# VinAIResearch/GaPro

Hardware: AMD Instinct MI355X
Metric: scenes/sec pseudo-label gen (ScanNetV2-train-shaped synthetic scenes) (higher is better)
Workload: dtype f64

## Files before the change

### gapro_amd/csrc/fit_wg.h

```cpp
#pragma once
#include <math.h>

#include <algorithm>
#include <type_traits>

#include "common.h"
#include "fit_layout.h"
#include "fit_math.h"
#include "epilogue.h"

namespace {
using namespace gapro_fit;
using namespace gapro_fit_math;

#ifndef GAPRO_NT
#define GAPRO_NT 512
#endif
constexpr int NT = GAPRO_NT;
constexpr int NW = NT / 64;
constexpr int kMaxMpLds = 512;
constexpr int kMaxDynLds = 150 * 1024;
constexpr int kRedSlots = 8;
constexpr int kTu4MinMp = 320;

using gapro_mfma::d4;



constexpr int kTileDoubles = NW * 16 * 17;
constexpr int kFuseMaxMp = 128;
constexpr int kWgTile = 128;
constexpr int kWgKC = 8;
constexpr int kWgRow = kWgTile + 16;
constexpr int kWgStage = 2 * kWgKC * kWgRow;
constexpr int kWgRingDoubles = 2 * kWgStage;
inline __host__ __device__ int part_doubles(int Mp) { return Mp <= kFuseMaxMp ? 3 * (Mp / 16) * Mp : 0; }
inline __host__ __device__ int scratch_doubles(int Mp) {
  const int a = kRedSlots * NT;
  const int b = Mp * 17 + 64 * 17;
  static_assert(kTileDoubles <= kWgStage, "the transpose tiles alias one stage of the operand ring");
  const int c = Mp <= kFuseMaxMp ? kTileDoubles + part_doubles(Mp) : kWgRingDoubles;
  int m = a > b ? a : b;
  return m > c ? m : c;
}
inline __host__ __device__ long long staged_lds_bytes(int m, int d) {
  const int Mp = gapro_pad_m(m, d);
  return 8LL * (2LL * d * Mp + scratch_doubles(Mp));
}
inline __host__ __device__ bool staged_ok(int m, int d) {
  return gapro_pad_m(m, d) <= kMaxMpLds && d <= 32 && staged_lds_bytes(m, d) <= kMaxDynLds;
}


struct Fit {
  int M, T, D, Mp;
  int M1;
  gd* mat[B_COUNT];
  gd* vec[V_COUNT];
  gd *X, *Z, *mZ, *vZ, *gZ, *Xt, *dinv, *dinvT, *scal;
};

#ifdef GAPRO_PROFILE
constexpr int kProfSlots = 28;
#endif
struct Shared {
  Fit f;
#ifdef GAPRO_PROFILE
  unsigned long long prof[kProfSlots];
  unsigned long long t_last;
  unsigned long long t_start;
#endif
  double red[NW];
  double dblk[16 * 17];
  double dinv[16 * 17];
  double c, rho_s, rho_l, s, ell, inv_l2;
  int status;
  int chol_bad;
};
__shared__ Shared g_sh;

#ifdef GAPRO_PROFILE
__device__ inline void prof_stamp(int id) {
  __syncthreads();
  if (threadIdx.x == 0) {
    const unsigned long long t = wall_clock64();
    g_sh.prof[id] += t - g_sh.t_last;
    g_sh.t_last = t;
  }
}
#else
__device__ inline void prof_stamp(int) {}
#endif

__device__ inline void gh_pair(double y, double mu, double sd, double t, double w, bool want_e, double* E, double* dmu,
                               double* dvar) {
  if (want_e) {
    double lp, r;
    log_ndtr_ratio_erfcx(y * (mu - sd * t), &lp, &r);
    *E += w * lp; *dmu += w * r; *dvar -= w * t * r;
    log_ndtr_ratio_erfcx(y * (mu + sd * t), &lp, &r);
    *E += w * lp; *dmu += w * r; *dvar += w * t * r;
  } else {
    double r = ndtr_ratio(y * (mu - sd * t));
    *dmu += w * r; *dvar -= w * t * r;
    r = ndtr_ratio(y * (mu + sd * t));
    *dmu += w * r; *dvar += w * t * r;
  }
}

__device__ inline int claim_fit(unsigned* ticket) {
  if (!ticket) return blockIdx.x;
  __shared__ int s_claim;
  if (threadIdx.x == 0) s_claim = (int)atomicAdd(ticket, 1u);
  __syncthreads();
  return __builtin_amdgcn_readfirstlane(s_claim);
}

__device__ inline double block_sum(double v) {
  v = wave_sum_shfl(v);
  __syncthreads();
  if ((threadIdx.x & 63) == 0) g_sh.red[threadIdx.x >> 6] = v;
  __syncthreads();
  double t = 0.0;
  for (int w = 0; w < NW; ++w) t += g_sh.red[w];
  return t;
}

__device__ inline double sqdist_t(const ldsd* At, int i, const ldsd* Bt, int j, int D, int Mp) {
  double s = 0.0;
  for (int d = 0; d < D; ++d) {
    const double t = At[d * Mp + i] - Bt[d * Mp + j];
    s += t * t;
  }
  return s;
}

__device__ inline void stage_points_t(ldsd* dst, const gd* src, int n, int D, int Mp) {
  for (int e = threadIdx.x; e < D * Mp; e += NT) {
    const int d = e / Mp, i = e - d * Mp;
    dst[e] = i < n ? src[(size_t)i * D + d] : 0.0;
  }
}

enum { ORD_ROWMAJOR = 0,
       ORD_ROWS_DESC = 1,
       ORD_COLMAJOR = 2,
       ORD_SHELLS = 3 };
typedef double d2 __attribute__((ext_vector_type(2)));
typedef __attribute__((address_space(3))) d2 lds_d2;
typedef __attribute__((address_space(1))) d2 g_d2;

template <int TU, bool SCALE, int KS = 2, int ORD = ORD_ROWMAJOR, bool TRIM = false, int PK = 0, int QK = 0,
          typename KRange, typename Epi>
__device__ __forceinline__ void gemm_tn_body(int mo_tiles, int no_tiles, bool lower_only, const gd* __restrict__ P,
                                          const gd* __restrict__ Q, int ld, const gd* __restrict__ qscale, KRange kr,
                                          Epi epi) {
  mo_tiles = uni(mo_tiles);
  no_tiles = uni(no_tiles);
  lower_only = uni((int)lower_only) != 0;
  ld = uni(ld);
  P = uni_ptr(P);
  Q = uni_ptr(Q);
  qscale = uni_ptr(qscale);
  const int wave = uni(threadIdx.x >> 6), lane = threadIdx.x & 63;
  const int lr = lane & 15, lq = lane >> 4;
  auto tile = [&](auto tv_tag, int i0, int j0) {
    constexpr int TV = decltype(tv_tag)::value;
    constexpr bool MINOR = PK || QK;
    constexpr int KSV = MINOR ? 2 : (TV >= 4 ? 1 : KS), KB = 4 * KSV;
    int klo, khi;
    kr(i0, j0, &klo, &khi);
    klo = uni(klo);
    khi = uni(khi);
    if (TRIM) {
      const int kmax = uni((g_sh.f.M + 7) / 8 * 8);
      khi = khi < kmax ? khi : kmax;
    }
    d4 acc[TV][TV];
#pragma unroll
    for (int u = 0; u < TV; ++u)
#pragma unroll
      for (int v = 0; v < TV; ++v) acc[u][v] = (d4){0.0, 0.0, 0.0, 0.0};
    const gd* pbase = PK ? P + (size_t)(i0 + lr) * ld + 2 * lq : P + (size_t)(MINOR ? 2 * lq : lq) * ld + i0 + lr;
    const gd* qbase = QK ? Q + (size_t)(j0 + lr) * ld + 2 * lq : Q + (size_t)(MINOR ? 2 * lq : lq) * ld + j0 + lr;
    double a0[KSV][TV], b0[KSV][TV], a1[KSV][TV], b1[KSV][TV];
    double s0[KSV], s1[KSV];
    auto load_block = [&](int k, double (&a)[KSV][TV], double (&b)[KSV][TV], double (&sc)[KSV]) {
      if constexpr (MINOR) {
#pragma unroll
        for (int u = 0; u < TV; ++u) {
          if constexpr (PK) {
            const d2 t = *(const g_d2*)(pbase + (size_t)(16 * u) * ld + k);
            a[0][u] = t[0];
            a[1][u] = t[1];
          } else {
            a[0][u] = pbase[(size_t)k * ld + 16 * u];
            a[1][u] = pbase[(size_t)(k + 1) * ld + 16 * u];
          }
        }
#pragma unroll
        for (int v = 0; v < TV; ++v) {
          if constexpr (QK) {
            const d2 t = *(const g_d2*)(qbase + (size_t)(16 * v) * ld + k);
            b[0][v] = t[0];
            b[1][v] = t[1];
          } else {
            b[0][v] = qbase[(size_t)k * ld + 16 * v];
            b[1][v] = qbase[(size_t)(k + 1) * ld + 16 * v];
          }
        }
        if (SCALE) {
          sc[0] = qscale[k + 2 * lq];
          sc[1] = qscale[k + 2 * lq + 1];
        }
      } else {
#pragma unroll
        for (int s = 0; s < KSV; ++s) {
          const gd* pr = pbase + (size_t)(k + 4 * s) * ld;
          const gd* qr = qbase + (size_t)(k + 4 * s) * ld;
#pragma unroll
          for (int u = 0; u < TV; ++u) a[s][u] = pr[16 * u];
#pragma unroll
          for (int v = 0; v < TV; ++v) b[s][v] = qr[16 * v];
          if (SCALE) sc[s] = qscale[k + 4 * s + lq];
        }
      }
    };
    auto mma_block = [&](double (&a)[KSV][TV], double (&b)[KSV][TV], double (&sc)[KSV]) {
#pragma unroll
      for (int s = 0; s < KSV; ++s) {
        double bs[TV];
#pragma unroll
        for (int v = 0; v < TV; ++v) bs[v] = SCALE ? b[s][v] * sc[s] : b[s][v];
#pragma unroll
        for (int u = 0; u < TV; ++u)
#pragma unroll
          for (int v = 0; v < TV; ++v)
            acc[u][v] = __builtin_amdgcn_mfma_f64_16x16x4f64(a[s][u], bs[v], acc[u][v], 0, 0, 0);
      }
    };
    if (klo < khi) {
      load_block(klo, a0, b0, s0);
      int k = klo;
#pragma nounroll
      for (; k + 2 * KB < khi; k += 2 * KB) {
        load_block(k + KB, a1, b1, s1);
        mma_block(a0, b0, s0);
        load_block(k + 2 * KB, a0, b0, s0);
        mma_block(a1, b1, s1);
      }
      if (k + KB < khi) {
        load_block(k + KB, a1, b1, s1);
        mma_block(a0, b0, s0);
        mma_block(a1, b1, s1);
      } else {
        mma_block(a0, b0, s0);
      }
    }
    run_epilogue<TV * TV>(epi, [&](int b, int* i, int* j) { *i = i0 + 16 * (b / TV); *j = j0 + 16 * (b % TV); },
                          [&](int b) -> const d4& { return acc[b / TV][b % TV]; });
  };
  constexpr int TE = TU >= 2 ? TU / 2 : TU;
  const int fo = TU >= 2 ? mo_tiles / 2 : mo_tiles, fn = TU >= 2 ? no_tiles / 2 : no_tiles;
  const int odd_i = TU >= 2 ? (mo_tiles & 1) : 0, odd_j = (TU >= 2 && !lower_only) ? (no_tiles & 1) : 0;
  const int nfull = lower_only ? fo * (fo + 1) / 2 : fo * fn;
  const int nrow = odd_i ? (lower_only ? mo_tiles : no_tiles) : 0;
  const int ncol = odd_j ? mo_tiles - odd_i : 0;
  const int ntiles = nfull + nrow + ncol;
  const int rounds = (ntiles + NW - 1) / NW;
#pragma nounroll
  for (int q = 0; q < rounds; ++q) {
    const int t = q * NW + ((q & 1) ? NW - 1 - wave : wave);
    if (t >= ntiles) continue;
    if (t >= nfull) {
      const int e = t - nfull;
      const int ih = e < nrow ? mo_tiles - 1 : e - nrow, jh = e < nrow ? e : no_tiles - 1;
      tile(std::integral_constant<int, TE>{}, 16 * TE * ih, 16 * TE * jh);
      continue;
    }
    int ti, tj;
    if (lower_only) {
      ti = 0;
      while ((ti + 1) * (ti + 2) / 2 <= t) ++ti;
      tj = t - ti * (ti + 1) / 2;
    } else if (ORD == ORD_ROWS_DESC) {
      ti = t / fn;
      tj = t - ti * fn;
      ti = fo - 1 - ti;
    } else if (ORD == ORD_COLMAJOR) {
      tj = t / fo;
      ti = t - tj * fo;
    } else if (ORD == ORD_SHELLS) {
      int m = 0;
      while ((m + 1) * (m + 1) <= t) ++m;
      const int r = t - m * m;
      ti = r <= m ? m : r - m - 1;
      tj = r <= m ? r : m;
    } else {
      ti = t / fn;
      tj = t - ti * fn;
    }
    tile(std::integral_constant<int, TU>{}, 16 * TU * ti, 16 * TU * tj);
  }
}

template <int TU, bool SCALE, int KS = 2, int ORD = ORD_ROWMAJOR, bool TRIM = false, int PK = 0, int QK = 0,
          typename KRange, typename Epi>
__device__ __noinline__ void gemm_tn(int mo_tiles, int no_tiles, bool lower_only, const gd* __restrict__ P,
                                     const gd* __restrict__ Q, int ld, const gd* __restrict__ qscale, KRange kr,
                                     Epi epi) {
  gemm_tn_body<TU, SCALE, KS, ORD, TRIM, PK, QK>(mo_tiles, no_tiles, lower_only, P, Q, ld, qscale, kr, epi);
}
template <int TU, bool SCALE, int KS = 2, int ORD = ORD_ROWMAJOR, bool TRIM = false, int PK = 0, int QK = 0,
          typename KRange, typename Epi>
__device__ __forceinline__ void gemm_tn_in(int mo_tiles, int no_tiles, bool lower_only, const gd* __restrict__ P,
                                        const gd* __restrict__ Q, int ld, const gd* __restrict__ qscale, KRange kr,
                                        Epi epi) {
  gemm_tn_body<TU, SCALE, KS, ORD, TRIM, PK, QK>(mo_tiles, no_tiles, lower_only, P, Q, ld, qscale, kr, epi);
}

template <bool SCALE, bool TRIM, int PF, typename KRange, typename Epi>
__device__ __noinline__ void gemm_wg(int rows16, int cols16, bool lower_only, const gd* __restrict__ P,
                                     const gd* __restrict__ Q, int ld, const gd* __restrict__ qscale, KRange kr,
                                     Epi epi, ldsd* ring) {
  static_assert(NT == 512 || !sizeof(Epi), "gemm_wg: eight waves, one k row of a chunk per wave");
  static_assert(PF == 2 || PF == 4, "gemm_wg: register stages");
  rows16 = uni(rows16);
  cols16 = uni(cols16);
  lower_only = uni((int)lower_only) != 0;
  ld = uni(ld);
  P = uni_ptr(P);
  Q = uni_ptr(Q);
  qscale = uni_ptr(qscale);
  const int wave = uni(threadIdx.x >> 6), lane = threadIdx.x & 63, lr = lane & 15, lq = lane >> 4;
  const int rows = 16 * rows16, cols = 16 * cols16;
  const int nti = (rows + kWgTile - 1) / kWgTile, ntj = (cols + kWgTile - 1) / kWgTile;
  const int wi = wave < 4 ? wave : 7 - wave, wj = wave >> 2;
  const int kmax = TRIM ? uni((g_sh.f.M + 7) / 8 * 8) : ld;
  const int lcol = 2 * lane;
  const int lds_wr = wave * kWgRow + lcol;
  const int fa = lq * kWgRow + 32 * wi + lr;
  const int fb = kWgKC * kWgRow + lq * kWgRow + 64 * wj + lr;
#pragma nounroll
  for (int ti = 0; ti < nti; ++ti) {
#pragma nounroll
    for (int tj = 0; tj < (lower_only ? ti + 1 : ntj); ++tj) {
      const int I0 = kWgTile * ti, J0 = kWgTile * tj;
      int klo = 1 << 30, khi = 0, plo = 1 << 30, phi = 0;
      unsigned on_mask = 0;
      if (rows - I0 >= kWgTile && cols - J0 >= kWgTile) {
        int lo, hi, d;
        kr(I0, J0, &lo, &d);
        kr(I0 + kWgTile - 16, J0 + kWgTile - 16, &d, &hi);
        hi = hi < kmax ? hi : kmax;
        if (lo < hi) { klo = lo; khi = hi; }
        const int pi0 = I0 + 32 * wi, pj0 = J0 + 64 * wj;
#pragma unroll
        for (int u = 0; u < 2; ++u)
#pragma unroll
          for (int v = 0; v < 4; ++v)
            if (!(lower_only && pi0 + 16 * u < pj0 + 16 * v)) on_mask |= 1u << (4 * u + v);
        if (on_mask) {
          kr(pi0, pj0, &lo, &d);
          kr(pi0 + 16, pj0 + 48, &d, &hi);
          hi = hi < kmax ? hi : kmax;
          if (lo < hi) { plo = lo; phi = hi; }
        }
      } else {
#pragma nounroll
        for (int bi = 0; bi < kWgTile / 16; ++bi) {
          const int ib = I0 + 16 * bi;
          if (ib >= rows) break;
#pragma nounroll
          for (int bj = 0; bj < kWgTile / 16; ++bj) {
            const int jb = J0 + 16 * bj;
            if (jb >= cols) break;
            if (lower_only && ib < jb) continue;
            const bool mine = (bi >> 1) == wi && (bj >> 2) == wj;
            if (mine) on_mask |= 1u << (4 * (bi & 1) + (bj & 3));
            int lo, hi;
            kr(ib, jb, &lo, &hi);
            hi = hi < kmax ? hi : kmax;
            if (lo >= hi) continue;
            klo = lo < klo ? lo : klo;
            khi = hi > khi ? hi : khi;
            if (mine) {
              plo = lo < plo ? lo : plo;
              phi = hi > phi ? hi : phi;
            }
          }
        }
      }
      klo = uni(klo) & ~(kWgKC - 1);
      khi = uni(khi);
      plo = uni(plo) & ~(kWgKC - 1);
      phi = uni(phi);
      on_mask = (unsigned)uni((int)on_mask);
      const int nch = klo < khi ? (khi - klo + kWgKC - 1) / kWgKC : 0;
      d4 acc[2][4];
#pragma unroll
      for (int u = 0; u < 2; ++u)
#pragma unroll
        for (int v = 0; v < 4; ++v) acc[u][v] = (d4){0.0, 0.0, 0.0, 0.0};
      if (nch > 0) {
        const bool pin = I0 + lcol < ld, qin = J0 + lcol < ld;
        const gd* pg = P + (size_t)wave * ld + (pin ? I0 + lcol : 0);
        const gd* qg = Q + (size_t)wave * ld + (qin ? J0 + lcol : 0);
        d2 rp[PF], rq[PF];
        double rs[PF];
        auto gload = [&](int n, d2& p, d2& q, double& sc) {
          n = n < nch ? n : nch - 1;
          const size_t o = (size_t)(klo + kWgKC * n) * ld;
          p = *(const g_d2*)(pg + o);
          q = *(const g_d2*)(qg + o);
          if (SCALE) sc = qscale[klo + kWgKC * n + wave];
        };
        auto lstore = [&](int stage, const d2& p, const d2& q, double sc) {
          ldsd* base = ring + stage * kWgStage + lds_wr;
          *(lds_d2*)base = p;
          *(lds_d2*)(base + kWgKC * kWgRow) = SCALE ? (d2){q[0] * sc, q[1] * sc} : q;
        };
        double fa0[2], fb0[4], fa1[2], fb1[4];
        auto rd = [&](int stage, int s, double (&a)[2], double (&b)[4]) {
          const ldsd* st = ring + stage * kWgStage + 4 * s * kWgRow;
#pragma unroll
          for (int v = 0; v < 4; ++v) b[v] = st[fb + 16 * v];
#pragma unroll
          for (int u = 0; u < 2; ++u) a[u] = st[fa + 16 * u];
        };
        auto mm = [&](int k0, const double (&a)[2], const double (&b)[4]) {
          if (k0 < plo || k0 >= phi) return;
#pragma unroll
          for (int u = 0; u < 2; ++u)
#pragma unroll
            for (int v = 0; v < 4; ++v)
              acc[u][v] = __builtin_amdgcn_mfma_f64_16x16x4f64(a[u], b[v], acc[u][v], 0, 0, 0);
        };
        auto chunk = [&](auto cur_tag, auto slot_tag, int c) {
          constexpr int CUR = decltype(cur_tag)::value, SLOT = decltype(slot_tag)::value;
          const int k0 = klo + kWgKC * c;
          lstore(CUR ^ 1, rp[SLOT], rq[SLOT], rs[SLOT]);
          gload(c + 1 + PF, rp[SLOT], rq[SLOT], rs[SLOT]);
          rd(CUR, 1, fa1, fb1);
          __builtin_amdgcn_sched_barrier(0);
          mm(k0, fa0, fb0);
          __builtin_amdgcn_sched_barrier(0);
          __syncthreads();
          rd(CUR ^ 1, 0, fa0, fb0);
          __builtin_amdgcn_sched_barrier(0);
          mm(k0, fa1, fb1);
          __builtin_amdgcn_sched_barrier(0);
        };
        using I0t = std::integral_constant<int, 0>;
        using I1t = std::integral_constant<int, 1>;
        using I2t = std::integral_constant<int, 2>;
        using I3t = std::integral_constant<int, 3>;
#pragma unroll
        for (int n = 0; n < PF; ++n) gload(n, rp[n], rq[n], rs[n]);
        lstore(0, rp[0], rq[0], rs[0]);
        gload(PF, rp[0], rq[0], rs[0]);
        __syncthreads();
        rd(0, 0, fa0, fb0);
        int c = 0;
        if constexpr (PF == 2) {
#pragma nounroll
          for (; c + 1 < nch; c += 2) {
            chunk(I0t{}, I1t{}, c);
            chunk(I1t{}, I0t{}, c + 1);
          }
          if (c < nch) chunk(I0t{}, I1t{}, c);
        } else {
#pragma nounroll
          for (; c + 3 < nch; c += 4) {
            chunk(I0t{}, I1t{}, c);
            chunk(I1t{}, I2t{}, c + 1);
            chunk(I0t{}, I3t{}, c + 2);
            chunk(I1t{}, I0t{}, c + 3);
          }
          if (c < nch) chunk(I0t{}, I1t{}, c);
          if (c + 1 < nch) chunk(I1t{}, I2t{}, c + 1);
          if (c + 2 < nch) chunk(I0t{}, I3t{}, c + 2);
        }
      }
      run_epilogue<8>(epi,
                      [&](int b, int* i, int* j) {
                        const bool on = (on_mask >> b) & 1u;
                        *i = on ? I0 + 32 * wi + 16 * (b >> 2) : -1;
                        *j = J0 + 64 * wj + 16 * (b & 3);
                      },
                      [&](int b) -> const d4& { return acc[b >> 2][b & 3]; });
    }
  }
}

__device__ inline void store_tile(const d4& v, gd* __restrict__ Cm, gd* __restrict__ CT, int ld, int i0, int j0,
                                  ldsd* tile ) {
  const int lane = threadIdx.x & 63, lr = lane & 15, lq = lane >> 4;
  if (Cm) {
#pragma unroll
    for (int r = 0; r < 4; ++r) Cm[(size_t)(i0 + lq + 4 * r) * ld + j0 + lr] = v[r];
  }
  if (CT) {
#pragma unroll
    for (int r = 0; r < 4; ++r) tile[(lq + 4 * r) * 17 + lr] = v[r];
    __builtin_amdgcn_fence(__ATOMIC_RELEASE, "wavefront", "local");
    __builtin_amdgcn_wave_barrier();
#pragma unroll
    for (int r = 0; r < 4; ++r) CT[(size_t)(j0 + lq + 4 * r) * ld + i0 + lr] = tile[lr * 17 + lq + 4 * r];
    __builtin_amdgcn_fence(__ATOMIC_ACQUIRE, "wavefront", "local");
    __builtin_amdgcn_wave_barrier();
  }
}

__device__ __noinline__ void diag_factor_invert(ldsd* panel, int kb) {
  const Fit& f = g_sh.f;
  const int Mp = f.Mp;
  kb = uni(kb);
  gd* LT = f.mat[B_LT];
  const int lane = threadIdx.x & 63, r = lane & 15;
#ifdef GAPRO_PROFILE
  const unsigned long long tp0 = wall_clock64();
#endif
  double rdiag[16];
  {
    double a[16];
#pragma unroll
    for (int c = 0; c < 16; ++c) a[c] = panel[r * 17 + c];
    bool bad = false;
#pragma unroll
    for (int j = 0; j < 16; ++j) {
      double d = lane_bcast(a[j], j);
      if (!(d > 0.0)) {
        bad = true;
        d = 1e-30;
      }
      const double rs = rsqrt(d);
      rdiag[j] = rs;
      const double lj = (r == j) ? d * rs : a[j] * rs;
      a[j] = lj;
#pragma unroll
      for (int c = j + 1; c < 16; ++c) a[c] -= lj * lane_bcast(lj, c);
    }
    if (bad && lane == 0) g_sh.chol_bad = 1;
    if (lane < 16) {
#pragma unroll
      for (int c = 0; c < 16; ++c) g_sh.dblk[r * 17 + c] = (c <= r) ? a[c] : 0.0;
    }
  }
  __builtin_amdgcn_fence(__ATOMIC_SEQ_CST, "wavefront", "local");
  __builtin_amdgcn_wave_barrier();
#ifdef GAPRO_PROFILE
  const unsigned long long tp1 = wall_clock64();
#endif
  {
    double x[16], b[16];
#pragma unroll
    for (int rr = 0; rr < 16; ++rr) b[rr] = (rr == r) ? 1.0 : 0.0;
#pragma unroll
    for (int q = 0; q < 16; ++q) {
      x[q] = (q >= r) ? b[q] * rdiag[q] : 0.0;
#pragma unroll
      for (int rr = q + 1; rr < 16; ++rr) b[rr] = fma(-g_sh.dblk[rr * 17 + q], x[q], b[rr]);
    }
    if (lane < 16) {
#pragma unroll
      for (int c = 0; c < 16; ++c) g_sh.dinv[c * 17 + r] = x[c];
    }
  }
  __builtin_amdgcn_fence(__ATOMIC_SEQ_CST, "wavefront", "local");
  __builtin_amdgcn_wave_barrier();
#ifdef GAPRO_PROFILE
  const unsigned long long tp2 = wall_clock64();
#endif
#pragma unroll
  for (int e = 0; e < 4; ++e) {
    const int idx = lane + 64 * e;
    const int rr = idx >> 4, cc = idx & 15;
    LT[(size_t)(16 * kb + rr) * Mp + 16 * kb + cc] = g_sh.dblk[cc * 17 + rr];
    f.dinv[(size_t)kb * 256 + idx] = g_sh.dinv[rr * 17 + cc];
    f.dinvT[(size_t)kb * 256 + idx] = g_sh.dinv[cc * 17 + rr];
  }
#ifdef GAPRO_PROFILE
  if (lane == 0) {
    const unsigned long long tp3 = wall_clock64();
    g_sh.prof[22] += tp1 - tp0;
    g_sh.prof[23] += tp2 - tp1;
    g_sh.prof[24] += tp3 - tp2;
  }
#endif
}

__device__ inline void chol_update_tile(d4& acc, const gd* pa, const gd* pb, int Mp, int Q) {
  const size_t st = (size_t)4 * Mp;
  auto ld = [&](int q, double (&a)[4], double (&b)[4]) {
    const size_t o = (size_t)q * Mp;
#pragma unroll
    for (int e = 0; e < 4; ++e) {
      a[e] = pa[o + e * st];
      b[e] = pb[o + e * st];
    }
  };
  auto mm = [&](double (&a)[4], double (&b)[4]) {
#pragma unroll
    for (int e = 0; e < 4; ++e) acc = __builtin_amdgcn_mfma_f64_16x16x4f64(-a[e], b[e], acc, 0, 0, 0);
  };
  if (Q <= 0) return;
  double a0[4], b0[4], a1[4], b1[4];
  ld(0, a0, b0);
  int q = 0;
#pragma nounroll
  for (; q + 32 < Q; q += 32) {
    ld(q + 16, a1, b1);
    mm(a0, b0);
    ld(q + 32, a0, b0);
    mm(a1, b1);
  }
  if (q + 16 < Q) {
    ld(q + 16, a1, b1);
    mm(a0, b0);
    mm(a1, b1);
  } else {
    mm(a0, b0);
  }
}

template <int DC>
__device__ __noinline__ void cholesky_fused(const ldsd* Zt, ldsd* panel, double s, double inv_l2, double jitter) {
  const Fit& f = g_sh.f;
  Shared& sh = g_sh;
  const int Mp = f.Mp, M = f.M, D = DC ? DC : f.D, nb = Mp / 16;
  gd* LT = f.mat[B_LT];
  const int wave = __builtin_amdgcn_readfirstlane(threadIdx.x >> 6), lane = threadIdx.x & 63;
  const int lr = lane & 15, lq = lane >> 4;
  for (int kb = 0; kb < nb; ++kb) {
    for (int ib = kb + wave; ib < nb; ib += NW) {
      d4 acc;
      const int col = 16 * kb + lr;
#pragma unroll
      for (int r = 0; r < 4; ++r) {
        const int row = 16 * ib + lq + 4 * r;
        double v = 0.0;
        if (row < M && col < M) {
          v = s * gapro_fit_math::rbf_exp(-0.5 * inv_l2 * sqdist_t(Zt, row, Zt, col, D, Mp));
          if (row == col) v += jitter;
        } else if (row == col) {
          v = 1.0;
        }
        acc[r] = v;
      }
      const gd* pa = LT + (size_t)lq * Mp + 16 * ib + lr;
      const gd* pb = LT + (size_t)lq * Mp + 16 * kb + lr;
      chol_update_tile(acc, pa, pb, Mp, 16 * kb);
      ldsd* dst = panel + (16 * (ib - kb)) * 17;
#pragma unroll
      for (int r = 0; r < 4; ++r) dst[(lq + 4 * r) * 17 + lr] = acc[r];
    }
    __syncthreads();
    prof_stamp(0);
    if (wave == 0) diag_factor_invert(panel, kb);
    __syncthreads();
    prof_stamp(5);
    const int rows_below = Mp - 16 * (kb + 1);
    ldsd* pb = panel + 16 * 17;
    for (int idx = threadIdx.x; idx < rows_below * 16; idx += NT) {
      const int i = idx >> 4, c = idx & 15;
      double acc = 0.0;
#pragma unroll
      for (int q = 0; q < 16; ++q) acc += (q <= c) ? pb[i * 17 + q] * sh.dinv[c * 17 + q] : 0.0;
      __builtin_amdgcn_fence(__ATOMIC_SEQ_CST, "wavefront", "local");
      __builtin_amdgcn_wave_barrier();
      pb[i * 17 + c] = acc;
    }
    __syncthreads();
    if (rows_below > 0)
      for (int idx = threadIdx.x; idx < rows_below * 16; idx += NT) {
        const int c = idx / rows_below, i = idx - c * rows_below;
        LT[(size_t)(16 * kb + c) * Mp + 16 * (kb + 1) + i] = pb[i * 17 + c];
      }
    __syncthreads();
    prof_stamp(18);
  }
}

inline __host__ __device__ int chol_panel_doubles(int Mp) { return Mp * 17 + 64 * 17; }
template <int DC>
__device__ __noinline__ void cholesky_fused_lookahead(const ldsd* Zt, ldsd* panels, double s, double inv_l2,
                                                      double jitter) {
  const Fit& f = g_sh.f;
  Shared& sh = g_sh;
  const int Mp = f.Mp, M = f.M, D = DC ? DC : f.D, nb = Mp / 16;
  gd* LT = f.mat[B_LT];
  const int wave = __builtin_amdgcn_readfirstlane(threadIdx.x >> 6), lane = threadIdx.x & 63;
  const int lr = lane & 15, lq = lane >> 4;
  const int PS = chol_panel_doubles(Mp);
  auto build = [&](int ib, int kb, int qb, ldsd* dst_panel) {
    d4 acc;
    const int col = 16 * kb + lr;
#pragma unroll
    for (int r = 0; r < 4; ++r) {
      const int row = 16 * ib + lq + 4 * r;
      double v = 0.0;
      if (row < M && col < M) {
        v = s * gapro_fit_math::rbf_exp(-0.5 * inv_l2 * sqdist_t(Zt, row, Zt, col, D, Mp));
        if (row == col) v += jitter;
      } else if (row == col) {
        v = 1.0;
      }
      acc[r] = v;
    }
    const gd* pa = LT + (size_t)lq * Mp + 16 * ib + lr;
    const gd* pb = LT + (size_t)lq * Mp + 16 * kb + lr;
    chol_update_tile(acc, pa, pb, Mp, 16 * qb);
    ldsd* dst = dst_panel + (16 * (ib - kb)) * 17;
#pragma unroll
    for (int r = 0; r < 4; ++r) dst[(lq + 4 * r) * 17 + lr] = acc[r];
  };
  for (int ib = wave; ib < nb; ib += NW) build(ib, 0, 0, panels);
  __syncthreads();
  for (int kb = 0; kb < nb; ++kb) {
    ldsd* cur = panels + (kb & 1) * PS;
    ldsd* nxt = panels + ((kb + 1) & 1) * PS;
    if (wave == 0) {
      if (NW <= 4) __builtin_amdgcn_s_setprio(3);
      diag_factor_invert(cur, kb);
      if (NW <= 4) __builtin_amdgcn_s_setprio(0);
    } else {
      for (int ib = kb + wave; ib < nb; ib += NW - 1) build(ib, kb + 1, kb, nxt);
    }
    __syncthreads();
    prof_stamp(5);
    const int rows_below = Mp - 16 * (kb + 1);
    ldsd* pb = cur + 16 * 17;
    for (int idx = threadIdx.x; idx < rows_below * 16; idx += NT) {
      const int i = idx >> 4, c = idx & 15;
      double acc = 0.0;
#pragma unroll
      for (int q = 0; q < 16; ++q) acc += (q <= c) ? pb[i * 17 + q] * sh.dinv[c * 17 + q] : 0.0;
      __builtin_amdgcn_fence(__ATOMIC_SEQ_CST, "wavefront", "local");
      __builtin_amdgcn_wave_barrier();
      pb[i * 17 + c] = acc;
    }
    __syncthreads();
    for (int ib = kb + 1 + wave; ib < nb; ib += NW) {
      ldsd* dst = nxt + (16 * (ib - kb - 1)) * 17;
      const ldsd* la = pb + (16 * (ib - kb - 1) + lr) * 17 + lq;
      const ldsd* lb = pb + lr * 17 + lq;
      d4 acc;
#pragma unroll
      for (int r = 0; r < 4; ++r) acc[r] = dst[(lq + 4 * r) * 17 + lr];
#pragma unroll
      for (int st = 0; st < 4; ++st) acc = __builtin_amdgcn_mfma_f64_16x16x4f64(-la[4 * st], lb[4 * st], acc, 0, 0, 0);
#pragma unroll
      for (int r = 0; r < 4; ++r) dst[(lq + 4 * r) * 17 + lr] = acc[r];
    }
    if (rows_below > 0)
      for (int idx = threadIdx.x; idx < rows_below * 16; idx += NT) {
        const int c = idx / rows_below, i = idx - c * rows_below;
        LT[(size_t)(16 * kb + c) * Mp + 16 * (kb + 1) + i] = pb[i * 17 + c];
      }
    __syncthreads();
    prof_stamp(18);
  }
}

template <int DC, int TMAX>
__device__ __noinline__ void cholesky_fused_lookahead_reg(const ldsd* Zt, ldsd* panel, double s, double inv_l2,
                                                          double jitter) {
  const Fit& f = g_sh.f;
  Shared& sh = g_sh;
  const int Mp = f.Mp, M = f.M, D = DC ? DC : f.D, nb = Mp / 16;
  gd* LT = f.mat[B_LT];
  const int wave = __builtin_amdgcn_readfirstlane(threadIdx.x >> 6), lane = threadIdx.x & 63;
  const int lr = lane & 15, lq = lane >> 4;
  auto build = [&](int ib, int kb, int qb) -> d4 {
    d4 acc;
    const int col = 16 * kb + lr;
#pragma unroll
    for (int r = 0; r < 4; ++r) {
      const int row = 16 * ib + lq + 4 * r;
      double v = 0.0;
      if (row < M && col < M) {
        v = s * gapro_fit_math::rbf_exp(-0.5 * inv_l2 * sqdist_t(Zt, row, Zt, col, D, Mp));
        if (row == col) v += jitter;
      } else if (row == col) {
        v = 1.0;
      }
      acc[r] = v;
    }
    const gd* pa = LT + (size_t)lq * Mp + 16 * ib + lr;
    const gd* pb = LT + (size_t)lq * Mp + 16 * kb + lr;
    chol_update_tile(acc, pa, pb, Mp, 16 * qb);
    return acc;
  };
  for (int ib = wave; ib < nb; ib += NW) {
    const d4 acc = build(ib, 0, 0);
    ldsd* dst = panel + (16 * ib) * 17;
#pragma unroll
    for (int r = 0; r < 4; ++r) dst[(lq + 4 * r) * 17 + lr] = acc[r];
  }
  __syncthreads();
  d4 nx[TMAX];
  for (int kb = 0; kb < nb; ++kb) {
    if (wave == 0) {
      diag_factor_invert(panel, kb);
    } else {
#pragma unroll
      for (int t = 0; t < TMAX; ++t) {
        const int ib = kb + wave + t * (NW - 1);
        if (ib < nb) nx[t] = build(ib, kb + 1, kb);
      }
    }
    __syncthreads();
    prof_stamp(5);
    const int rows_below = Mp - 16 * (kb + 1);
    ldsd* pb = panel + 16 * 17;
    for (int idx = threadIdx.x; idx < rows_below * 16; idx += NT) {
      const int i = idx >> 4, c = idx & 15;
      double acc = 0.0;
#pragma unroll
      for (int q = 0; q < 16; ++q) acc += (q <= c) ? pb[i * 17 + q] * sh.dinv[c * 17 + q] : 0.0;
      __builtin_amdgcn_fence(__ATOMIC_SEQ_CST, "wavefront", "local");
      __builtin_amdgcn_wave_barrier();
      pb[i * 17 + c] = acc;
    }
    __syncthreads();
    if (wave != 0) {
#pragma unroll
      for (int t = 0; t < TMAX; ++t) {
        const int ib = kb + wave + t * (NW - 1);
        if (ib < nb) {
          const ldsd* la = pb + (16 * (ib - kb - 1) + lr) * 17 + lq;
          const ldsd* lb = pb + lr * 17 + lq;
#pragma unroll
          for (int st = 0; st < 4; ++st)
            nx[t] = __builtin_amdgcn_mfma_f64_16x16x4f64(-la[4 * st], lb[4 * st], nx[t], 0, 0, 0);
        }
      }
    }
    if (rows_below > 0)
      for (int idx = threadIdx.x; idx < rows_below * 16; idx += NT) {
        const int c = idx / rows_below, i = idx - c * rows_below;
        LT[(size_t)(16 * kb + c) * Mp + 16 * (kb + 1) + i] = pb[i * 17 + c];
      }
    __syncthreads();
    if (wave != 0) {
#pragma unroll
      for (int t = 0; t < TMAX; ++t) {
        const int ib = kb + wave + t * (NW - 1);
        if (ib < nb) {
          ldsd* dst = panel + (16 * (ib - kb - 1)) * 17;
#pragma unroll
          for (int r = 0; r < 4; ++r) dst[(lq + 4 * r) * 17 + lr] = nx[t][r];
        }
      }
    }
    __syncthreads();
    prof_stamp(18);
  }
}

template <int DC, int LOOKAHEAD>
__device__ __noinline__ void cholesky_psd_safe(const ldsd* Zt, ldsd* scratch, double s, double inv_l2, double jitter,
                                               int retries, double psd_jitter) {
  double extra = 0.0;
  for (int attempt = 0;; ++attempt) {
    if (LOOKAHEAD == 1) cholesky_fused_lookahead<DC>(Zt, scratch, s, inv_l2, jitter + extra);
    else if (LOOKAHEAD == 2) cholesky_fused_lookahead_reg<DC, 3>(Zt, scratch, s, inv_l2, jitter + extra);
    else if (LOOKAHEAD == 3) cholesky_fused_lookahead_reg<DC, 5>(Zt, scratch, s, inv_l2, jitter + extra);
    else cholesky_fused<DC>(Zt, scratch, s, inv_l2, jitter + extra);
    const int bad = g_sh.chol_bad;
    if (!bad) return;
    __syncthreads();
    if (threadIdx.x == 0) {
      g_sh.chol_bad = 0;
      if (attempt >= retries) g_sh.status = GAPRO_ERR_CHOLESKY;
    }
    __syncthreads();
    if (attempt >= retries) return;
    extra = psd_jitter * pow(10.0, (double)attempt);
  }
}

template <int CNT>
__device__ inline void inv_column(int k, ldsd* tile) {
  const Fit& f = g_sh.f;
  const int Mp = f.Mp;
  const gd* LT = f.mat[B_LT];
  gd* LI = f.mat[B_LI];
  gd* U = f.mat[B_U];
  const int lane = threadIdx.x & 63, lr = lane & 15, lq = lane >> 4;
  constexpr int MAXR = CNT > 1 ? CNT - 1 : 1;
  d4 blk[CNT];
  double A0[MAXR * 4], A1[MAXR * 4], D0[4], D1[4];
  auto ldrow = [&](int ii, double (&A)[MAXR * 4], double (&D)[4]) {
    const int i = k + ii;
#pragma unroll
    for (int jj = 0; jj < MAXR; ++jj)
      if (jj < ii) {
        const gd* pa = LT + (size_t)(16 * (k + jj) + lq) * Mp + 16 * i + lr;
#pragma unroll
        for (int st = 0; st < 4; ++st) A[jj * 4 + st] = pa[(size_t)(4 * st) * Mp];
      }
#pragma unroll
    for (int st = 0; st < 4; ++st) D[st] = f.dinvT[(size_t)i * 256 + (4 * st + lq) * 16 + lr];
  };
  d4 dk;
#pragma unroll
  for (int r = 0; r < 4; ++r) dk[r] = f.dinv[(size_t)k * 256 + (lq + 4 * r) * 16 + lr];
  if (CNT > 1) ldrow(1, A1, D1);
  store_tile(dk, LI, U, Mp, 16 * k, 16 * k, tile);
  blk[0] = dk;
#pragma unroll
  for (int ii = 1; ii < CNT; ++ii) {
    if (ii + 1 < CNT) {
      if ((ii + 1) & 1) ldrow(ii + 1, A1, D1);
      else ldrow(ii + 1, A0, D0);
    }
    d4 acc = (d4){0.0, 0.0, 0.0, 0.0};
#pragma unroll
    for (int jj = 0; jj < MAXR; ++jj)
      if (jj < ii) {
#pragma unroll
        for (int st = 0; st < 4; ++st)
          acc = __builtin_amdgcn_mfma_f64_16x16x4f64((ii & 1) ? A1[jj * 4 + st] : A0[jj * 4 + st], blk[jj][st], acc, 0, 0, 0);
      }
    d4 out = (d4){0.0, 0.0, 0.0, 0.0};
#pragma unroll
    for (int st = 0; st < 4; ++st)
      out = __builtin_amdgcn_mfma_f64_16x16x4f64(-((ii & 1) ? D1[st] : D0[st]), acc[st], out, 0, 0, 0);
    store_tile(out, LI, U, Mp, 16 * (k + ii), 16 * k, tile);
    blk[ii] = out;
  }
}
__device__ __noinline__ void tri_inverse_strip(ldsd* tiles) {
  const int nb = g_sh.f.Mp / 16;
  const int wave = __builtin_amdgcn_readfirstlane(threadIdx.x >> 6);
  ldsd* tile = tiles + wave * 16 * 17;
  for (int k = wave; k < nb; k += NW) {
    switch (nb - k) {
      case 1: inv_column<1>(k, tile); break;
      case 2: inv_column<2>(k, tile); break;
      case 3: inv_column<3>(k, tile); break;
      case 4: inv_column<4>(k, tile); break;
#if GAPRO_NT >= 320
      case 5: inv_column<5>(k, tile); break;
      case 6: inv_column<6>(k, tile); break;
      case 7: inv_column<7>(k, tile); break;
      default: inv_column<8>(k, tile); break;
#else
      default: break;
#endif
    }
  }
}

template <int NBR>
__device__ __noinline__ void tri_inverse(ldsd* tiles) {
  const Fit& f = g_sh.f;
  const int Mp = f.Mp, nb = Mp / 16;
  const gd* LT = f.mat[B_LT];
  gd* LI = f.mat[B_LI];
  gd* U = f.mat[B_U];
  const int wave = __builtin_amdgcn_readfirstlane(threadIdx.x >> 6), lane = threadIdx.x & 63;
  const int lr = lane & 15, lq = lane >> 4;
  ldsd* tile = tiles + wave * 16 * 17;
  unsigned long long mine = 0;
  if (NBR == 0) {
    int load[NW];
#pragma unroll
    for (int w = 0; w < NW; ++w) load[w] = 0;
    for (int k = 0; k < nb; ++k) {
      int best = 0;
#pragma unroll
      for (int w = 1; w < NW; ++w) best = load[w] < load[best] ? w : best;
      const int n = nb - k;
#pragma unroll
      for (int w = 0; w < NW; ++w) load[w] += (w == best) ? n * (n - 1) / 2 + 1 : 0;
      if (best == wave) mine |= 1ull << k;
    }
  }
  for (int k = NBR > 0 ? wave : 0; k < nb; k += NBR > 0 ? NW : 1) {
    if (NBR == 0 && !((mine >> k) & 1ull)) continue;
    d4 blk[NBR > 0 ? NBR : 1];
    d4 dk;
#pragma unroll
    for (int r = 0; r < 4; ++r) dk[r] = f.dinv[(size_t)k * 256 + (lq + 4 * r) * 16 + lr];
    store_tile(dk, LI, U, Mp, 16 * k, 16 * k, tile);
    if (NBR > 0) blk[0] = dk;
    if (NBR > 0) {
#pragma unroll
      for (int ii = 1; ii < NBR; ++ii) {
        const int i = k + ii;
        if (i < nb) {
          d4 acc = (d4){0.0, 0.0, 0.0, 0.0};
#pragma unroll
          for (int jj = 0; jj < ii; ++jj) {
            const gd* pa = LT + (size_t)(16 * (k + jj) + lq) * Mp + 16 * i + lr;
#pragma unroll
            for (int sstep = 0; sstep < 4; ++sstep)
              acc = __builtin_amdgcn_mfma_f64_16x16x4f64(pa[(size_t)(4 * sstep) * Mp], blk[jj][sstep], acc, 0, 0, 0);
          }
          d4 out = (d4){0.0, 0.0, 0.0, 0.0};
#pragma unroll
          for (int sstep = 0; sstep < 4; ++sstep) {
            const double a = -f.dinvT[(size_t)i * 256 + (4 * sstep + lq) * 16 + lr];
            out = __builtin_amdgcn_mfma_f64_16x16x4f64(a, acc[sstep], out, 0, 0, 0);
          }
          store_tile(out, LI, U, Mp, 16 * i, 16 * k, tile);
          blk[ii] = out;
        }
      }
    } else {
      for (int i = k + 1; i < nb; ++i) {
        d4 nacc = (d4){0.0, 0.0, 0.0, 0.0};
        __builtin_amdgcn_fence(__ATOMIC_SEQ_CST, "workgroup");
        chol_update_tile(nacc, LT + (size_t)(16 * k + lq) * Mp + 16 * i + lr, LI + (size_t)(16 * k + lq) * Mp + 16 * k + lr,
                         Mp, 16 * (i - k));
        d4 out = (d4){0.0, 0.0, 0.0, 0.0};
#pragma unroll
        for (int sstep = 0; sstep < 4; ++sstep) {
          const double a = f.dinvT[(size_t)i * 256 + (4 * sstep + lq) * 16 + lr];
          out = __builtin_amdgcn_mfma_f64_16x16x4f64(a, nacc[sstep], out, 0, 0, 0);
        }
        store_tile(out, LI, U, Mp, 16 * i, 16 * k, tile);
      }
    }
  }
}

struct ColMap {
  int G, col, grp;
  bool active;
};
__device__ inline ColMap col_map(int Mp) {
  ColMap c;
  c.G = NT / Mp;
  c.col = threadIdx.x % Mp;
  c.grp = threadIdx.x / Mp;
  c.active = c.grp < c.G;
  return c;
}

template <int DC>
__device__ __noinline__ void build_kx(const ldsd* Zt, const ldsd* Pt, int ncols, double s, double inv_l2) {
  const Fit& f = g_sh.f;
  const int Mp = f.Mp, M = f.M, D = DC ? DC : f.D;
  gd* KX = f.mat[B_KX];
  const ColMap cm = col_map(Mp);
  if (!cm.active) return;
  const int n = cm.col;
  for (int k = cm.grp; k < Mp; k += cm.G) {
    double v = 0.0;
    if (k < M && n < ncols) v = s * gapro_fit_math::rbf_exp(-0.5 * inv_l2 * sqdist_t(Zt, k, Pt, n, D, Mp));
    KX[(size_t)k * Mp + n] = v;
  }
}

__device__ __noinline__ void mean_var(double s, double jitter, ldsd* red) {
  const Fit& f = g_sh.f;
  const int Mp = f.Mp;
  const gd* A = f.mat[B_A];
  const gd* BM = f.mat[B_BM];
  const gd* m = f.vec[V_M];
  const ColMap cm = col_map(Mp);
  double pm = 0.0, pv = 0.0;
  if (cm.active) {
    for (int i = cm.grp; i < Mp; i += cm.G) {
      const double a = A[(size_t)i * Mp + cm.col], b = BM[(size_t)i * Mp + cm.col];
      pm += m[i] * a;
      pv += b * b - a * a;
    }
  }
  red[threadIdx.x] = pm;
  red[NT + threadIdx.x] = pv;
  __syncthreads();
  if (threadIdx.x < Mp) {
    double sm = 0.0, sv = 0.0;
    for (int g = 0; g < cm.G; ++g) {
      sm += red[g * Mp + threadIdx.x];
      sv += red[NT + g * Mp + threadIdx.x];
    }
    f.vec[V_MU][threadIdx.x] = sm;
    f.vec[V_VAR][threadIdx.x] = s + jitter + sv;
  }
  __syncthreads();
}

__device__ __noinline__ void weighted_colsum(const gd* Mtx, const gd* w, int Mp, gd* out, ldsd* red) {
  const ColMap cm = col_map(Mp);
  double p = 0.0;
  if (cm.active)
    for (int r = cm.grp; r < Mp; r += cm.G) p += w[r] * Mtx[(size_t)r * Mp + cm.col];
  red[threadIdx.x] = p;
  __syncthreads();
  if (threadIdx.x < Mp) {
    double sacc = 0.0;
    for (int g = 0; g < cm.G; ++g) sacc += red[g * Mp + threadIdx.x];
    out[threadIdx.x] = sacc;
  }
  __syncthreads();
}

__device__ __noinline__ double quadrature(double c, double min_variance, double Nd, bool want_e, ldsd* red,
                                          double* g_c, double* gv_sum) {
  const Fit& f = g_sh.f;
  const int Mp = f.Mp, M = f.M;
  gd* gmu = f.vec[V_GMU];
  gd* gv = f.vec[V_GV];
  double e_tot = 0.0, gc_part = 0.0, gvs_part = 0.0;
  constexpr int PPR = NT / 10;
  const int q = threadIdx.x % 10, nl = threadIdx.x / 10;
  for (int n0 = 0; n0 < M; n0 += PPR) {
    const int n = n0 + nl;
    double E = 0.0, dmu = 0.0, dvar = 0.0;
    const bool on = nl < PPR && n < M;
    if (on) {
      const double mu = f.vec[V_MU][n] + c;
      const double vraw = f.vec[V_VAR][n];
      const double var = vraw < min_variance ? min_variance : vraw;
      const double sd = sqrt(2.0 * var);
      const double y = n < f.M1 ? -1.0 : 1.0;
      const double t = c_gh_t[q], w = c_gh_w[q];
      gh_pair(y, mu, sd, t, w, want_e, &E, &dmu, &dvar);
    }
    red[threadIdx.x] = E;
    red[NT + threadIdx.x] = dmu;
    red[2 * NT + threadIdx.x] = dvar;
    __syncthreads();
    if (on && q == 0) {
      double se = 0.0, sm = 0.0, sv = 0.0;
      for (int qq = 0; qq < 10; ++qq) {
        se += red[threadIdx.x + qq];
        sm += red[NT + threadIdx.x + qq];
        sv += red[2 * NT + threadIdx.x + qq];
      }
      const double ipi = 0.56418958354775628695;
      const double vraw = f.vec[V_VAR][n];
      const bool clamped = vraw < min_variance;
      const double var = clamped ? min_variance : vraw;
      const double y = n < f.M1 ? -1.0 : 1.0;
      const double g1 = -(ipi * sm * y) / Nd;
      const double g2 = clamped ? 0.0 : -(ipi * sv * y / sqrt(2.0 * var)) / Nd;
      gmu[n] = g1;
      gv[n] = g2;
      e_tot += ipi * se;
      gc_part += g1;
      gvs_part += g2;
    }
    __syncthreads();
  }
  for (int n = M + threadIdx.x; n < Mp; n += NT) {
    gmu[n] = 0.0;
    gv[n] = 0.0;
  }
  *g_c = block_sum(gc_part);
  *gv_sum = block_sum(gvs_part);
  return want_e ? block_sum(e_tot) : 0.0;
}

template <int DMAX, bool ZX, int U, int DC>
__device__ __noinline__ void kernel_grads_adam_z(ldsd* Zt, const ldsd* Xt, const gd* Gm, const gd* GTm,
                                                 const gd* GKXT, double s, double inv_l2, double step_size,
                                                 double bc2s, ldsd* red, double* gs_out, double* gl_out,
                                                 const ldsd* zx_rows = nullptr) {
  const Fit& f = g_sh.f;
  const int Mp = f.Mp, M = f.M, D = DC ? DC : f.D;
  const ColMap cm = col_map(Mp);
  const int j = cm.col;
  double acc[DMAX];
#pragma unroll
  for (int d = 0; d < DMAX; ++d) acc[d] = 0.0;
  double gs = 0.0, gl = 0.0;
  if (DMAX > 8) {
    double wsum = 0.0;
    if (cm.active && j < M) {
      for (int i = cm.grp; i < M; i += cm.G) {
        const size_t o = (size_t)i * Mp + j;
        const double gsym = 0.5 * (Gm[o] + GTm[o]);
        const double g3 = ZX ? GKXT[o] : 0.0;
        double d2 = 0.0, d2x = 0.0;
#pragma unroll 8
        for (int d = 0; d < D; ++d) {
          const double zjd = Zt[d * Mp + j];
          const double a = zjd - Zt[d * Mp + i];
          d2 += a * a;
          if (ZX) {
            const double bx = zjd - Xt[d * Mp + i];
            d2x += bx * bx;
          }
        }
        const double e = gapro_fit_math::rbf_exp(-0.5 * inv_l2 * d2);
        const double w = gsym * s * e;
        gs += gsym * e;
        gl += w * d2;
        double wx = 0.0;
        if (ZX) {
          const double ex = gapro_fit_math::rbf_exp(-0.5 * inv_l2 * d2x);
          wx = g3 * s * ex;
          gs += g3 * ex;
          gl += wx * d2x;
        }
        wsum += 2.0 * w + wx;
#pragma unroll
        for (int d = 0; d < DMAX; ++d)
          if (d < D) acc[d] += 2.0 * w * Zt[d * Mp + i] + (ZX ? wx * Xt[d * Mp + i] : 0.0);
      }
    }
#pragma unroll
    for (int d = 0; d < DMAX; ++d) acc[d] = (d < D) ? wsum * Zt[d * Mp + j] - acc[d] : 0.0;
  } else if (cm.active && j < M) {
    double zj[DMAX];
#pragma unroll
    for (int d = 0; d < DMAX; ++d) zj[d] = (d < D) ? Zt[d * Mp + j] : 0.0;
    for (int i0 = cm.grp; i0 < M; i0 += cm.G * U) {
      double g1[U], g2[U], g3[U];
#pragma unroll
      for (int u = 0; u < U; ++u) {
        const int i = i0 + u * cm.G;
        const bool act = i < M;
        const size_t o = (size_t)(act ? i : 0) * Mp + j;
        g1[u] = act ? Gm[o] : 0.0;
        g2[u] = act ? GTm[o] : 0.0;
        g3[u] = (ZX && act) ? GKXT[o] : 0.0;
      }
#pragma unroll
      for (int u = 0; u < U; ++u) {
        const int i = i0 + u * cm.G;
        if (u * cm.G >= M) break;
        if (i < M) {
          double t[DMAX];
          double d2 = 0.0;
#pragma unroll
          for (int d = 0; d < DMAX; ++d) {
            t[d] = (d < D) ? zj[d] - Zt[d * Mp + i] : 0.0;
            d2 += t[d] * t[d];
          }
          const double e = gapro_fit_math::rbf_exp(-0.5 * inv_l2 * d2);
          const double gsym = 0.5 * (g1[u] + g2[u]);
          const double w = gsym * s * e;
          gs += gsym * e;
          gl += w * d2;
#pragma unroll
          for (int d = 0; d < DMAX; ++d) acc[d] += 2.0 * w * t[d];
          if (ZX) {
            double d2x = 0.0;
#pragma unroll
            for (int d = 0; d < DMAX; ++d) {
              t[d] = (d < D) ? zj[d] - Xt[d * Mp + i] : 0.0;
              d2x += t[d] * t[d];
            }
            const double ex = gapro_fit_math::rbf_exp(-0.5 * inv_l2 * d2x);
            const double wx = g3[u] * s * ex;
            gs += g3[u] * ex;
            gl += wx * d2x;
#pragma unroll
            for (int d = 0; d < DMAX; ++d) acc[d] += wx * t[d];
          }
        }
      }
    }
  }
  prof_stamp(20);
  *gs_out = block_sum(gs);
  *gl_out = block_sum(gl);
  prof_stamp(21);
  const double b1 = 0.9, b2 = 0.999, aeps = 1e-8;
#pragma unroll
  for (int dc = 0; dc < DMAX; dc += kRedSlots) {
    if (dc < D) {
#pragma unroll
      for (int e = 0; e < kRedSlots; ++e)
        if (dc + e < DMAX) red[e * NT + threadIdx.x] = acc[dc + e];
      __syncthreads();
      if (threadIdx.x < M) {
#pragma unroll
        for (int e = 0; e < kRedSlots; ++e) {
          const int d = dc + e;
          if (d < D && d < DMAX) {
            double sacc = 0.0;
            for (int g = 0; g < cm.G; ++g) sacc += red[e * NT + g * Mp + threadIdx.x];
            const size_t zi = (size_t)threadIdx.x * D + d;
            if (!ZX) sacc += zx_rows ? zx_rows[threadIdx.x * 8 + d] : f.gZ[zi];
            const double grad = -inv_l2 * sacc;
            f.gZ[zi] = grad;
            const double m1 = b1 * f.mZ[zi] + (1.0 - b1) * grad;
            const double m2 = b2 * f.vZ[zi] + (1.0 - b2) * grad * grad;
            f.mZ[zi] = m1;
            f.vZ[zi] = m2;
            const double znew = f.Z[zi] - step_size * m1 / (sqrt(m2) / bc2s + aeps);
            f.Z[zi] = znew;
            Zt[d * Mp + threadIdx.x] = znew;
          }
        }
      }
      __syncthreads();
    }
  }
}

template <int WG, int TU, bool SCALE, int ORD, int PK = 0, int QK = 0, typename KRange, typename Epi>
__device__ inline void product(int mo, int no, bool lower, const gd* __restrict__ P, const gd* __restrict__ Q, int ld,
                               const gd* __restrict__ qs, KRange kr, Epi epi, ldsd* ring) {
  if constexpr (WG == 0) {
    gemm_tn_in<TU, SCALE, 2, ORD, true, PK, QK>(mo, no, lower, P, Q, ld, qs, kr, epi);
  } else {
    const int rows = (16 * mo + 31) / 32 * 32, cols = (16 * no + 31) / 32 * 32;
    const int R = rows / kWgTile * kWgTile, Cc = cols / kWgTile * kWgTile;
    constexpr bool kMajor = !(PK || QK);
    if constexpr (kMajor) {
      if (R > 0 && Cc > 0 && !lower) gemm_wg<SCALE, true, WG>(R / 16, Cc / 16, false, P, Q, ld, qs, kr, epi, ring);
    }
    auto strip_t = [&](auto tu_tag, int r0, int c0, int nr, int nc, bool low) {
      constexpr int TUS = decltype(tu_tag)::value;
      if (nr <= 0 || nc <= 0) return;
      gemm_tn_in<TUS, SCALE, 2, ORD_ROWMAJOR, true, PK, QK>(
          nr / (8 * TUS), nc / (8 * TUS), low, PK ? P + (size_t)r0 * ld : P + r0, QK ? Q + (size_t)c0 * ld : Q + c0, ld, qs,
          [=](int i0, int j0, int* lo, int* hi) {
            int l0, h0, l1, h1;
            kr(r0 + i0, c0 + j0, &l0, &h0);
            kr(r0 + i0 + 16 * TUS - 16, c0 + j0 + 16 * TUS - 16, &l1, &h1);
            *lo = l0;
            *hi = h1;
          },
          shifted_epi(epi, r0, c0));
    };
    auto strip = [&](int r0, int c0, int nr, int nc, bool low) {
      strip_t(std::integral_constant<int, 2>{}, r0, c0, nr, nc, low);
    };
    if (lower) {
      if constexpr (WG == 4) {
        if (rows >= 352) {
          strip_t(std::integral_constant<int, 4>{}, 0, 0, rows, cols, true);
          return;
        }
      }
      strip(0, 0, rows, cols, true);
      return;
    }
    if constexpr (kMajor) {
      strip(R, 0, rows - R, cols, false);
      strip(0, Cc, R, cols - Cc, false);
    } else {
      strip(0, 0, rows, cols, false);
    }
  }
}

__device__ inline void fit_setup(const gapro_fit_desc& desc, int D, const float* __restrict__ feats_spp,
                                 const int* __restrict__ idx, const double* __restrict__ init_mean,
                                 double* __restrict__ ws, ldsd* Zt, ldsd* Pt) {
  Shared& sh = g_sh;
  Fit& f = sh.f;
  const Layout lay = make_layout(desc.m1 + desc.m2, desc.t, D);
  gd* base = (gd*)(ws + desc.ws_offset);
  if (threadIdx.x == 0) {
    f.M = desc.m1 + desc.m2;
    f.M1 = desc.m1;
    f.T = desc.t;
    f.D = D;
    f.Mp = lay.Mp;
    for (int b = 0; b < B_COUNT; ++b) f.mat[b] = base + lay.mat + (long long)b * lay.Mp * lay.Mp;
    for (int v = 0; v < V_COUNT; ++v) f.vec[v] = base + lay.vec + (long long)v * lay.Mp;
    f.X = base + lay.xz;
    f.Z = f.X + (long long)lay.Mp * D;
    f.mZ = f.Z + (long long)lay.Mp * D;
    f.vZ = f.mZ + (long long)lay.Mp * D;
    f.gZ = f.vZ + (long long)lay.Mp * D;
    f.Xt = base + lay.xt;
    f.dinv = base + lay.dinv;
    f.dinvT = f.dinv + (long long)lay.Mp * 16;
    f.scal = base + lay.scal;
    sh.c = 0.0;
    sh.rho_s = 0.0;
    sh.rho_l = 0.0;
    sh.status = GAPRO_OK;
    sh.chol_bad = 0;
#ifdef GAPRO_PROFILE
    for (int i = 0; i < kProfSlots; ++i) sh.prof[i] = 0;
    sh.t_last = wall_clock64();
    sh.t_start = sh.t_last;
#endif
  }
  const int M = desc.m1 + desc.m2, Mp = lay.Mp;
  for (long long i = threadIdx.x; i < lay.total; i += NT) base[i] = 0.0;
  __syncthreads();
  const int* my_idx = idx + desc.idx_offset;
  for (int e = threadIdx.x; e < M * D; e += NT) {
    const int i = e / D, d = e - i * D;
    const double v = (double)feats_spp[(size_t)my_idx[i] * D + d];
    f.X[e] = v;
    f.Z[e] = v;
  }
  for (int e = threadIdx.x; e < desc.t * D; e += NT) {
    const int i = e / D, d = e - i * D;
    f.Xt[e] = (double)feats_spp[(size_t)my_idx[M + i] * D + d];
  }
  for (int i = threadIdx.x; i < M; i += NT) {
    f.vec[V_Y][i] = i < desc.m1 ? -1.0 : 1.0;
    f.vec[V_M][i] = init_mean ? init_mean[desc.idx_offset + i] : 0.0;
    f.mat[B_LS][(size_t)i * Mp + i] = 1.0;
    f.mat[B_LST][(size_t)i * Mp + i] = 1.0;
  }
  __syncthreads();
  stage_points_t(Zt, f.Z, M, D, Mp);
  stage_points_t(Pt, f.X, M, D, Mp);
  __syncthreads();
}

__device__ inline void fit_epilogue(const gapro_fit_desc& desc, const gapro_fit_options& opt, int* o_status,
                                    double* o_loss) {
  __syncthreads();
  if (threadIdx.x == 0) {
    int st = g_sh.status;
    if (st == GAPRO_OK && !isfinite(o_loss[desc.slot]) && opt.training_iter > 0) st = GAPRO_ERR_NOT_FINITE;
    o_status[desc.slot] = st;
    g_sh.f.scal[S_STATUS] = (double)st;
  }
}

}
```

### gapro_amd/csrc/svgp_fit_small.hip

```cpp
#define GAPRO_NT 256
#define k_svgp_fit_strip k_svgp_fit_strip256
#include "fit_strip.h"

long long gapro_fit_strip_small_lds_bytes(int m, int feat_dim) { return strip_lds_bytes(m, feat_dim); }

int gapro_launch_fit_strip_small(hipStream_t stream, int n_fits, int n_wg, unsigned* d_ticket, int feat_dim,
                                 size_t lds_bytes, const float* d_feats_spp, const int* d_idx,
                                 const gapro_fit_desc* d_descs, const double* d_init_mean,
                                 const gapro_fit_options& opt, double* d_workspace, float* d_probs, float* d_probs_new,
                                 unsigned char* d_labels, float* d_mu, float* d_var, int* d_fit_status,
                                 double* d_fit_loss) {
  return launch_fit_strip(stream, n_fits, n_wg, d_ticket, feat_dim, lds_bytes, d_feats_spp, d_idx, d_descs,
                          d_init_mean, opt, d_workspace, d_probs, d_probs_new, d_labels, d_mu, d_var, d_fit_status,
                          d_fit_loss);
}
```

Before: 379.4.

## Split diagonal block factor and inverse across waves with LDS step flags

The 16x16 diagonal block Cholesky factorisation and its triangular inversion, previously done serially by wave 0, are split: wave 0 factors and publishes each column to LDS with a step counter, while the last wave spin-waits on that counter and computes the inverse column by column in parallel. The global stores of the diagonal factor and inverse move after the trailing update, done by all threads. This aims to shorten the serial critical path per panel step, at the cost of spin-waiting on one wave that would otherwise build panels. It is disabled for the 256-thread small variant.

```diff
diff --git a/gapro_amd/csrc/fit_wg.h b/gapro_amd/csrc/fit_wg.h
--- a/gapro_amd/csrc/fit_wg.h
+++ b/gapro_amd/csrc/fit_wg.h
@@ -73,9 +73,11 @@
   double red[NW];
   double dblk[16 * 17];
   double dinv[16 * 17];
+  double rdiag[16];
   double c, rho_s, rho_l, s, ell, inv_l2;
   int status;
   int chol_bad;
+  int diag_step;
 };
 __shared__ Shared g_sh;
 
@@ -590,6 +592,100 @@
 #endif
 }
 
+#ifndef GAPRO_DIAG_SPLIT
+#define GAPRO_DIAG_SPLIT 1
+#endif
+constexpr bool kDiagSplit = GAPRO_DIAG_SPLIT != 0 && NW >= 3;
+typedef __attribute__((address_space(3))) int ldsi;
+
+__device__ __noinline__ void diag_factor_publish(ldsd* panel, int kb) {
+  kb = uni(kb);
+  const int lane = threadIdx.x & 63, r = lane & 15;
+#ifdef GAPRO_PROFILE
+  const unsigned long long tp0 = wall_clock64();
+#endif
+  ldsd* pub = (lane == 16) ? (ldsd*)g_sh.rdiag : (ldsd*)g_sh.dblk + r * 17;
+  ldsi* step = (ldsi*)&g_sh.diag_step;
+  double a[16];
+#pragma unroll
+  for (int c = 0; c < 16; ++c) a[c] = panel[r * 17 + c];
+  bool bad = false;
+#pragma unroll
+  for (int j = 0; j < 16; ++j) {
+    double d = lane_bcast(a[j], j);
+    if (!(d > 0.0)) {
+      bad = true;
+      d = 1e-30;
+    }
+    const double rs = rsqrt(d);
+    const double lj = (r == j) ? d * rs : a[j] * rs;
+    a[j] = lj;
+    pub[j] = (lane == 16) ? rs : (j <= r) ? lj : 0.0;
+#pragma unroll
+    for (int c = j + 1; c < 16; ++c) a[c] -= lj * lane_bcast(lj, c);
+    __builtin_amdgcn_fence(__ATOMIC_RELEASE, "workgroup", "local");
+    __hip_atomic_store(step, 16 * kb + j + 1, __ATOMIC_RELAXED, __HIP_MEMORY_SCOPE_WORKGROUP);
+  }
+  if (bad && lane == 0) g_sh.chol_bad = 1;
+#ifdef GAPRO_PROFILE
+  if (lane == 0) g_sh.prof[22] += wall_clock64() - tp0;
+#endif
+}
+
+__device__ __noinline__ void diag_invert_trailing(int kb) {
+  kb = uni(kb);
+  const int lane = threadIdx.x & 63, r = lane & 15;
+  const ldsd* dblk = (const ldsd*)g_sh.dblk;
+  const ldsd* rd = (const ldsd*)g_sh.rdiag;
+  ldsi* step = (ldsi*)&g_sh.diag_step;
+#ifdef GAPRO_PROFILE
+  unsigned long long tq = 0;
+#endif
+  double x[16], b[16];
+#pragma unroll
+  for (int rr = 0; rr < 16; ++rr) b[rr] = (rr == r) ? 1.0 : 0.0;
+#pragma unroll
+  for (int q = 0; q < 16; ++q) {
+    while (uni(__hip_atomic_load(step, __ATOMIC_RELAXED, __HIP_MEMORY_SCOPE_WORKGROUP)) < 16 * kb + q + 1) {
+      if (NW <= 4) __builtin_amdgcn_s_sleep(1);
+    }
+    __builtin_amdgcn_fence(__ATOMIC_ACQUIRE, "workgroup", "local");
+#ifdef GAPRO_PROFILE
+    if (q == 15) tq = wall_clock64();
+#endif
+    x[q] = (q >= r) ? b[q] * rd[q] : 0.0;
+#pragma unroll
+    for (int rr = q + 1; rr < 16; ++rr) b[rr] = fma(-dblk[rr * 17 + q], x[q], b[rr]);
+  }
+  if (lane < 16) {
+#pragma unroll
+    for (int c = 0; c < 16; ++c) g_sh.dinv[c * 17 + r] = x[c];
+  }
+  __builtin_amdgcn_fence(__ATOMIC_SEQ_CST, "wavefront", "local");
+  __builtin_amdgcn_wave_barrier();
+#ifdef GAPRO_PROFILE
+  if (lane == 0) g_sh.prof[23] += wall_clock64() - tq;
+#endif
+}
+
+__device__ inline void diag_store_global(int kb) {
+  const Fit& f = g_sh.f;
+  const int Mp = f.Mp;
+  gd* LT = f.mat[B_LT];
+#ifdef GAPRO_PROFILE
+  const unsigned long long ts0 = wall_clock64();
+#endif
+  for (int idx = threadIdx.x; idx < 256; idx += NT) {
+    const int rr = idx >> 4, cc = idx & 15;
+    LT[(size_t)(16 * kb + rr) * Mp + 16 * kb + cc] = g_sh.dblk[cc * 17 + rr];
+    f.dinv[(size_t)kb * 256 + idx] = g_sh.dinv[rr * 17 + cc];
+    f.dinvT[(size_t)kb * 256 + idx] = g_sh.dinv[cc * 17 + rr];
+  }
+#ifdef GAPRO_PROFILE
+  if (threadIdx.x == 0) g_sh.prof[24] += wall_clock64() - ts0;
+#endif
+}
+
 __device__ inline void chol_update_tile(d4& acc, const gd* pa, const gd* pb, int Mp, int Q) {
   const size_t st = (size_t)4 * Mp;
   auto ld = [&](int q, double (&a)[4], double (&b)[4]) {
@@ -716,15 +812,18 @@
     for (int r = 0; r < 4; ++r) dst[(lq + 4 * r) * 17 + lr] = acc[r];
   };
   for (int ib = wave; ib < nb; ib += NW) build(ib, 0, 0, panels);
+  if (kDiagSplit && threadIdx.x == 0) g_sh.diag_step = 0;
   __syncthreads();
   for (int kb = 0; kb < nb; ++kb) {
     ldsd* cur = panels + (kb & 1) * PS;
     ldsd* nxt = panels + ((kb + 1) & 1) * PS;
     if (wave == 0) {
       if (NW <= 4) __builtin_amdgcn_s_setprio(3);
-      diag_factor_invert(cur, kb);
+      if (kDiagSplit) diag_factor_publish(cur, kb);
+      else diag_factor_invert(cur, kb);
       if (NW <= 4) __builtin_amdgcn_s_setprio(0);
     } else {
+      if (kDiagSplit && wave == NW - 1) diag_invert_trailing(kb);
       for (int ib = kb + wave; ib < nb; ib += NW - 1) build(ib, kb + 1, kb, nxt);
     }
     __syncthreads();
@@ -753,6 +852,7 @@
 #pragma unroll
       for (int r = 0; r < 4; ++r) dst[(lq + 4 * r) * 17 + lr] = acc[r];
     }
+    if (kDiagSplit) diag_store_global(kb);
     if (rows_below > 0)
       for (int idx = threadIdx.x; idx < rows_below * 16; idx += NT) {
         const int c = idx / rows_below, i = idx - c * rows_below;
diff --git a/gapro_amd/csrc/svgp_fit_small.hip b/gapro_amd/csrc/svgp_fit_small.hip
--- a/gapro_amd/csrc/svgp_fit_small.hip
+++ b/gapro_amd/csrc/svgp_fit_small.hip
@@ -1,4 +1,7 @@
 #define GAPRO_NT 256
+#ifndef GAPRO_DIAG_SPLIT
+#define GAPRO_DIAG_SPLIT 0
+#endif
 #define k_svgp_fit_strip k_svgp_fit_strip256
 #include "fit_strip.h"
 
```

After: 382.1 (median of 2 runs). Within noise of the previous version (+0.7%).
